# lunarlab-gatech/MorphSym-HGNN

Measured on AMD Instinct MI355X. Metric: graph-windows/sec fwd+bwd, A1-C2 GRF regression, higher is better.
Workload: dtype bf16; 1 GPU; A1-C2 GRF regression (3-D), h=128, L=3, T=150, 8192 windows/GPU, fwd+MSE+bwd, all parameter gradients; global_batch=8192, parallelism=dp1, rccl_ranks=0

## Files before the change

morphsym_hgnn_amd/csrc/mshgnn.hip:

```cpp
#include "mshgnn_slab.hpp"
extern "C" const char* mshgnn_last_error(void) { return g_err.c_str(); }
extern "C" const char* mshgnn_version(void) { return "mshgnn 0.5 (gfx950)"; }
extern "C" int mshgnn_abi_version(void) { return MSHGNN_ABI_VERSION; }
extern "C" size_t mshgnn_struct_size(int which) {
    switch (which) {
        case 0: return sizeof(mshgnn_desc);
        case 1: return sizeof(mshgnn_info);
        case 2: return sizeof(mshgnn_ws_layout);
        case 3: return sizeof(mshgnn_window_desc);
        case 4: return sizeof(mshgnn_kernel_stat);
        default: return 0;
    }
}


template <typename T> __device__ __forceinline__ void prep_one(const PrepArgs& a, int idx, bool with_bias) {
    constexpr int EPC = Prec<T>::EPC, NBV = Prec<T>::NBV;
    const int vec_per_pack = H * H / EPC;
    const int npk = a.pack_n < 0 ? a.n_packs : a.pack_n;
    const int total = npk * vec_per_pack;
    if (idx < total) {
        const int pack = a.pack0 + idx / vec_per_pack, r = idx % vec_per_pack;
        const int gid = pack * vec_per_pack + r;
        const int lane = r % 64, v = (r / 64) % NBV, wv = r / (64 * NBV);
// ... 14 lines not shown
                    else g[i][x] = a.params[pd.src[i] + (int64_t)k * pd.ld + col];
                }
            }
#pragma unroll
        for (int x = 0; x < EPC; ++x) {
            float sum = 0.f;
#pragma unroll
            for (int i = 0; i < 8; ++i) sum += g[i][x];
            out[x] = from_f32<T>(sum);
        }
        T* dst = reinterpret_cast<T*>(a.wpack) + (size_t)gid * EPC;
#pragma unroll
        for (int x = 0; x < EPC; ++x) dst[x] = out[x];
    } else if (with_bias) {
        const int b = idx - total;
        if (b < a.n_biases * H) {
            const BiasDesc bd = a.biases[b / H];
            float s = 0.f;
            for (int i = 0; i < bd.n_src; ++i) s += a.params[bd.src[i] + (b % H)];
            a.bias[b] = s;
        }
    }
}
template <typename T> __global__ void k_prep(PrepArgs a) { prep_one<T>(a, blockIdx.x * blockDim.x + threadIdx.x, true); }


__device__ __forceinline__ u32x4 splice8(u32x4 A, u32x4 B, int n0) {
    const unsigned __int128 a = ((unsigned __int128)(((unsigned long long)A[3] << 32) | A[2]) << 64) | (((unsigned long long)A[1] << 32) | A[0]);
    const unsigned __int128 b = ((unsigned __int128)(((unsigned long long)B[3] << 32) | B[2]) << 64) | (((unsigned long long)B[1] << 32) | B[0]);
    const int sh = 16 * n0;
    const unsigned __int128 r = (a & ((((unsigned __int128)1) << sh) - 1)) | (b << sh);
    return u32x4{(unsigned)r, (unsigned)(r >> 32), (unsigned)(r >> 64), (unsigned)(r >> 96)};
}
template <typename T, bool ALIGNED, bool SERIES = false, int SRC = 0, bool NORM = false> __global__ __launch_bounds__(256) void k_enc_fwd(EncArgs a, SeriesSrc ser, WideSrc wsrc) {
    using P = Prec<T>;
    static_assert(!NORM || SERIES, "standardisation is part of the series gather");
    static_assert(!SERIES || (sizeof(T) == 2 && ALIGNED), "the series gather is a bf16 path");
    static_assert(SRC == 0 || (sizeof(T) == 2 && ALIGNED && !SERIES), "wide source rows: bf16 plan, aligned destination rows");
    constexpr int MB = P::ENC_MB;
    constexpr int VPB = P::ROWS * P::CPR, NIT = VPB / 256 > 0 ? VPB / 256 : 1, BPP = 256 / VPB > 0 ? 256 / VPB : 1;
    extern __shared__ __attribute__((aligned(16))) char smem[];
    const int tid = threadIdx.x, lane = tid & 63, wv = __builtin_amdgcn_readfirstlane(tid >> 6);
    const int lab_blocks = SERIES ? (int)((ser.lab.B + 255) / 256) : 0;
    if constexpr (SERIES) {
        if ((int)blockIdx.x < lab_blocks) {
            const int64_t b = (int64_t)blockIdx.x * 256 + tid;
            if (b < ser.lab.B) window_labels_one(ser.lab, b);
            return;
        }
    }
    const int bid = (int)blockIdx.x - lab_blocks;
    if (bid >= a.wg_prefix[a.n_types]) {
        if constexpr (sizeof(T) == 2 && ALIGNED && !SERIES) prep_one<T>(a.prep, (bid - a.wg_prefix[a.n_types]) * 256 + tid, false);
        return;
    }
    int t = 0;
    while (t + 1 < a.n_types && bid >= a.wg_prefix[t + 1]) ++t;
    const int local = bid - a.wg_prefix[t];
    const int node = a.node_list[a.node_off[t] + (ENC_ORDER ? local % a.nodes[t] : local / a.tiles)], tile = ENC_ORDER ? local / a.nodes[t] : local % a.tiles;
    const bool skip = SERIES && ((a.skip_mask >> (a.tbase[t] + node)) & 1ull) != 0;
    const int w0 = tile * MB * P::ROWS;
    const T* x = reinterpret_cast<const T*>(a.x[t]);
    const int64_t pitch = a.pitch[t];
    const int F = a.width[t], nt = a.tbase[t + 1] - a.tbase[t], nkc = a.nkc[t], vb = a.vb[t];
    const uint8_t* sg = a.signs + a.sign_off[t] + (size_t)node * nkc * H;
    const T* wpack = reinterpret_cast<const T*>(a.wpack);
    const float* bias = a.bias + (size_t)max(a.bias_idx[t], 0) * H;

    typename P::Acc acc[MB];
#pragma unroll
    for (int m = 0; m < MB; ++m) acc_init_bias<T>(acc[m], bias, wv, lane);
    const int c = tid % P::CPR, r0 = (tid % VPB) / P::CPR, sub = tid / VPB;
    typename P::BFrag bf;
    typename P::AFrag af;
    const AOff<T> ao(lane);
    u32x4 v[MB / BPP][NIT];
    u32x4 rawv[(SERIES || SRC) ? MB / BPP : 1][NIT];
    u32x2 wv8[SRC ? MB / BPP : 1][SRC ? SRC : 1];
    const bool unit_ok = SRC == 8 || (F & 1) == 0;
    const int64_t spitch = SRC ? wsrc.pitch[t] : 0;
    int srow[SERIES ? MB / BPP : 1];
    u32x4 vn[NORM ? MB / BPP : 1][2];
    RunStats rsa[NORM ? MB / BPP : 1], rsb[NORM ? MB / BPP : 1];
    int n_n0 = 8; bool n_has_a = false, n_has_b = false;
    __shared__ unsigned long long rp_s[SERIES ? 16 : 1];
    int rfirst = 0, rend = 0;
    if constexpr (SERIES) {
#pragma unroll
        for (int mi = 0; mi < MB / BPP; ++mi) srow[mi] = (int)ser.starts[min(w0 + (mi * BPP + sub) * P::ROWS + r0, a.B - 1)];
        rfirst = ser.rows[2 * (ser.row0[t] + node)]; rend = ser.rows[2 * (ser.row0[t] + node) + 1];
        if (tid < 16) rp_s[tid] = rfirst + tid < rend ? ser.run_ptr[rfirst + tid] : 0ull;
        __syncthreads();
    }
    auto fetch = [&](int kc) {
        const int k0 = kc * H + c * P::EPC;
        const int nvalid = min(P::EPC, F - k0);
        if constexpr (SERIES) {
            const int j = k0 / ser.T, off = k0 - j * ser.T, n0 = min(P::EPC, ser.T - off);
            const bool second = nvalid > n0;
            auto run_ptr_of = [&](int jj) -> unsigned long long { return jj < 16 ? rp_s[jj] : (rfirst + jj < rend ? ser.run_ptr[rfirst + jj] : 0ull); };
            const unsigned long long pa = nvalid > 0 ? run_ptr_of(j) : 0ull, pb = second ? run_ptr_of(j + 1) : 0ull;
            if constexpr (NORM) {
                n_n0 = n0; n_has_a = pa != 0ull; n_has_b = pb != 0ull;
                const u32x4 ones32 = u32x4{0x3f800000u, 0x3f800000u, 0x3f800000u, 0x3f800000u};
#pragma unroll
                for (int mi = 0; mi < MB / BPP; ++mi) {
                    u32x4 a0 = nvalid > 0 ? ones32 : u32x4{0, 0, 0, 0}, a1 = a0;
                    const double* sp2 = ser.stats + ((size_t)min(w0 + (mi * BPP + sub) * P::ROWS + r0, a.B - 1) * ser.n_runs + rfirst + j) * 2;
                    rsa[mi] = RunStats{0.0, 1.0}; rsb[mi] = RunStats{0.0, 1.0};
                    if (pa) {
                        const float* sp = reinterpret_cast<const float*>(pa) + srow[mi] + off;
                        a0 = *reinterpret_cast<const u32x4*>(sp); a1 = *reinterpret_cast<const u32x4*>(sp + 4);
                        const f64x2 sv = *reinterpret_cast<const f64x2*>(sp2);
                        rsa[mi] = RunStats{sv[0], sv[1]};
                    }
                    if (second) {
                        u32x4 b0 = ones32, b1 = ones32;
                        if (pb) {
                            const float* sp = reinterpret_cast<const float*>(pb) + srow[mi];
                            b0 = *reinterpret_cast<const u32x4*>(sp); b1 = *reinterpret_cast<const u32x4*>(sp + 4);
                            const f64x2 sv = *reinterpret_cast<const f64x2*>(sp2 + 2);
                            rsb[mi] = RunStats{sv[0], sv[1]};
                        }
                        splice8f(a0, a1, b0, b1, n0);
                    }
                    vn[mi][0] = a0; vn[mi][1] = a1;
                }
                return;
            }
            const u32x4 ones = u32x4{0x3f803f80u, 0x3f803f80u, 0x3f803f80u, 0x3f803f80u};
#pragma unroll
            for (int mi = 0; mi < MB / BPP; ++mi) {
                u32x4 va = nvalid > 0 ? ones : u32x4{0, 0, 0, 0};
                if (pa) va = *reinterpret_cast<const u32x4*>(reinterpret_cast<const T*>(pa) + srow[mi] + off);
                if (second) {
                    u32x4 vb2 = ones;
                    if (pb) vb2 = *reinterpret_cast<const u32x4*>(reinterpret_cast<const T*>(pb) + srow[mi]);
                    va = splice8(va, vb2, n0);
                }
                v[mi][0] = va;
            }
            return;
        }
        if constexpr (SRC > 0) {
#pragma unroll
            for (int mi = 0; mi < MB / BPP; ++mi) {
                const int w = w0 + (mi * BPP + sub) * P::ROWS + r0;
                const char* row = reinterpret_cast<const char*>(wsrc.p[t]) + ((size_t)min(w, a.B - 1) * nt + node) * spitch * SRC;
                wide_fetch<SRC>(wv8[mi], row, k0, F, unit_ok, w < a.B);
            }
            return;
        }
#pragma unroll
        for (int mi = 0; mi < MB / BPP; ++mi)
#pragma unroll
            for (int it = 0; it < NIT; ++it) {
                const int m = mi * BPP + sub, row = r0 + it * (256 / P::CPR), w = w0 + m * P::ROWS + row;
                if constexpr (ALIGNED) {
                    const T* src = x + ((size_t)min(w, a.B - 1) * nt + node) * pitch + (nvalid > 0 ? k0 : kc * H);
                    v[mi][it] = ld16<ENC_NT>(src);
                } else {
                    v[mi][it] = u32x4{0, 0, 0, 0};
                    if (w < a.B) v[mi][it] = load_chunk<T>(x + ((size_t)w * nt + node) * pitch + k0, nvalid, vb);
                }
            }
    };
    fetch(0);
    for (int kc = 0; kc < nkc; ++kc) {
        const u32x4 sx = sign_xor<T>(sg + kc * H + c * P::EPC);
        const int nv = F - (kc * H + c * P::EPC);
        __syncthreads();
#pragma unroll
        for (int mi = 0; mi < MB / BPP; ++mi)
#pragma unroll
            for (int it = 0; it < NIT; ++it) {
                u32x4 raw;
                if constexpr (SRC > 0) {
                    f32x4 lo4, hi4;
                    wide_to_f32<SRC>(wv8[mi], nv, lo4, hi4);
                    raw = pack_oct(lo4, hi4);
                } else if constexpr (NORM) {
                    u32x4 a0 = vn[mi][0], a1 = vn[mi][1];
                    standardise_oct(a0, a1, n_n0, n_has_a, n_has_b, rsa[mi], rsb[mi]);
                    raw = pack_oct(__builtin_bit_cast(f32x4, a0), __builtin_bit_cast(f32x4, a1));
                    if (kc + 1 == nkc) raw = chunk_keep_first<T>(raw, nv);
                } else
                raw = kc + 1 == nkc ? chunk_keep_first<T>(v[mi][it], nv) : v[mi][it];
                *reinterpret_cast<u32x4*>(smem + lds_chunk<T>(mi * BPP + sub, r0 + it * (256 / P::CPR), c)) = raw ^ sx;
                if constexpr (SERIES || SRC > 0) rawv[mi][it] = raw;
            }
        __syncthreads();
        if (!skip) load_bfrag<T>(bf, wpack, a.pack0[t] + kc, wv, lane);
        if (kc + 1 < nkc) fetch(kc + 1);
        if constexpr (SERIES || SRC > 0) {
#pragma unroll
            for (int mi = 0; mi < MB / BPP; ++mi)
#pragma unroll
                for (int it = 0; it < NIT; ++it) {
                    const int w = w0 + (mi * BPP + sub) * P::ROWS + r0 + it * (256 / P::CPR), k0 = kc * H + c * P::EPC;
                    if (x != nullptr && w < a.B && k0 < (int)pitch) *reinterpret_cast<u32x4*>(const_cast<T*>(x) + ((size_t)w * nt + node) * pitch + k0) = rawv[mi][it];
                }
        }
        if (!skip) {
#pragma unroll
            for (int m = 0; m < MB; ++m) {
                if (w0 + m * P::ROWS < a.B) {
                    load_afrag<T>(af, smem, m, ao);
                    mac(acc[m], af, bf);
                }
            }
        }
    }
    if (skip) return;
    T* x0 = reinterpret_cast<T*>(a.x0);
    const int gnode = a.tbase[t] + node;
#pragma unroll
    for (int m = 0; m < MB; ++m) {
        const int w = w0 + m * P::ROWS + c_win(lane);
        if (w0 + m * P::ROWS < a.B) {
            const unsigned bits = relu_with_bits<T>(acc[m]);
            if (a.mask0) a.mask0[relu_tile_base(gnode, a.B, (w0 + m * P::ROWS) >> 4, wv) + lane] = (uint8_t)bits;
        }
        if (w < a.B) store_oct(x0 + act_idx(w, gnode, a.B) + wv * 32 + c_oct(lane), acc[m].c[0], acc[m].c[1]);
    }
}

struct LayerArgs {
    const void* x_in;
    void* x_out;
    unsigned* maskbits;
    void* hb; void* t1;
    void* dh; void* du;
    const void* x_act;
    const void* wpack; const float* bias; const int* prog;
    int B, NN, n_mlp;
    int dbg;
};

template <typename T>
__device__ __forceinline__ void store_relu_bits(const typename Prec<T>::Acc& acc, unsigned* maskbits, int NN, int n, int w0, int B, int wn, int lane) {
    unsigned bits = 0;
#pragma unroll
    for (int fb = 0; fb < 2; ++fb)
// ... 1404 lines not shown
            p->hp.d = *desc;
        }
        *out = p;
        return MSHGNN_OK;
    }
    int ndev = 0;
    if (hipGetDeviceCount(&ndev) != hipSuccess || ndev == 0) {
        delete p; return set_err(MSHGNN_EHIP, "no HIP device: the MS-HGNN engine has no CPU fallback");
    }
#ifdef MSHGNN_ABLATE
    { const char* e = getenv("MSHGNN_DBG"); p->dbg = e ? atoi(e) : 0; e = getenv("MSHGNN_DBG_GW"); p->dbg_gw = e ? atoi(e) : 0; }
#endif
    HostPlan& hp = p->hp;
    auto up = [&](void** dptr, const void* src, size_t bytes) -> int {
        HIPCHK(hipMalloc(dptr, std::max<size_t>(bytes, 16)));
        if (bytes) HIPCHK(hipMemcpy(*dptr, src, bytes, hipMemcpyHostToDevice));
        return MSHGNN_OK;
    };
    int rc;
    if ((rc = up((void**)&p->d_tables, hp.tables.data(), hp.tables.size() * 4)) != 0 ||
        (rc = up((void**)&p->d_signs, hp.signs.data(), hp.signs.size())) != 0 ||
        (rc = up((void**)&p->d_out_mask, hp.out_mask_f.data(), hp.out_mask_f.size() * 4)) != 0 ||
        (rc = up((void**)&p->d_packs, hp.packs.data(), hp.packs.size() * sizeof(PackDesc))) != 0 ||
        (rc = up((void**)&p->d_biases, hp.biases.data(), hp.biases.size() * sizeof(BiasDesc))) != 0) {
        mshgnn_plan_destroy(p); return rc;
    }
    const int lds = hp.n_blk * hp.blk_bytes;
    if (hp.d.dtype == MSHGNN_BF16X3) {
        p->use_fused = true;
        { const char* et = getenv("MSHGNN_STEP_KERNEL"); p->use_step = !(et && atoi(et) == 0); }
        if ((rc = x3_set_attrs(p))) { mshgnn_plan_destroy(p); return rc; }
    } else if (hp.d.dtype == MSHGNN_F32) {
        if ((rc = set_lds_attr(k_layer_fwd<float>, lds)) || (rc = set_lds_attr(k_layer_bwd<float>, lds)) ||
            (rc = set_lds_attr(k_enc_fwd<float, true>, Prec<float>::ENC_MB * Prec<float>::BLK)) || (rc = set_lds_attr(k_enc_fwd<float, false>, Prec<float>::ENC_MB * Prec<float>::BLK))) { mshgnn_plan_destroy(p); return rc; }
    } else {
        if ((rc = set_lds_attr(k_layer_fwd<__bf16>, lds)) || (rc = set_lds_attr(k_layer_bwd<__bf16>, lds)) ||
            (rc = set_lds_attr(k_enc_fwd<__bf16, true>, Prec<__bf16>::ENC_MB * Prec<__bf16>::BLK)) || (rc = set_lds_attr(k_enc_fwd<__bf16, true, true>, Prec<__bf16>::ENC_MB * Prec<__bf16>::BLK)) || (rc = set_lds_attr(k_enc_fwd<__bf16, true, false, 8>, Prec<__bf16>::ENC_MB * Prec<__bf16>::BLK)) || (rc = set_lds_attr(k_enc_fwd<__bf16, true, false, 4>, Prec<__bf16>::ENC_MB * Prec<__bf16>::BLK)) || (rc = set_lds_attr(k_enc_fwd<__bf16, false>, Prec<__bf16>::ENC_MB * Prec<__bf16>::BLK))) { mshgnn_plan_destroy(p); return rc; }
        const char* e = getenv("MSHGNN_FUSED");
        p->use_fused = hp.fused && !(e && atoi(e) == 0);
        if (p->use_fused) {
            const int flds = (hp.fs_blk + FS_EXTRA_BLK) * Prec<__bf16>::BLK;
            if ((rc = set_lds_attr(k_stack_fwd<__bf16>, flds)) || (rc = set_lds_attr(k_stack_bwd<__bf16>, flds)) || (rc = set_lds_attr(k_stack_step<__bf16>, flds))) { mshgnn_plan_destroy(p); return rc; }
            const char* es = getenv("MSHGNN_SLAB");
            p->use_slab = hp.slab && !(es && atoi(es) == 0);
            p->slab_force = es && atoi(es) == 2;
            { int dev = 0, cus = 256; if (hipGetDevice(&dev) == hipSuccess) (void)hipDeviceGetAttribute(&cus, hipDeviceAttributeMultiprocessorCount, dev); p->n_cu = cus > 0 ? cus : 256; }
            if (p->use_slab && ((rc = set_lds_attr(slab_fwd_kernel(hp), flds)) || (rc = set_lds_attr(slab_bwd_kernel(hp), flds)) ||
                                (rc = set_lds_attr(slab_step_kernel(hp), flds)))) { mshgnn_plan_destroy(p); return rc; }
            { const char* esp = getenv("MSHGNN_SPEC"); p->use_spec = p->use_slab && !(esp && atoi(esp) == 0); }
            if (p->use_spec && (rc = set_spec_attrs(p, flds))) { mshgnn_plan_destroy(p); return rc; }
            { const char* et = getenv("MSHGNN_STEP_KERNEL"); p->use_step = !(et && atoi(et) == 0); }

            { const char* eg = TUNE_ENV("MSHGNN_STAGGER"); p->stagger = eg ? atoi(eg) : 0; }
        }
    }
    *out = p;
    return MSHGNN_OK;
}

extern "C" void mshgnn_plan_destroy(mshgnn_plan* p) {
    if (!p) return;
    gen_destroy(p);
    if (p->d_tables) (void)hipFree(p->d_tables);
    if (p->d_signs) (void)hipFree(p->d_signs);
    if (p->d_out_mask) (void)hipFree(p->d_out_mask);
    if (p->d_packs) (void)hipFree(p->d_packs);
    if (p->d_biases) (void)hipFree(p->d_biases);
    if (p->d_ig_nodes) (void)hipFree(p->d_ig_nodes);
    for (ProfRec& r : p->recs) { (void)hipEventDestroy(r.a); (void)hipEventDestroy(r.b); }
    for (hipEvent_t e : p->free_events) (void)hipEventDestroy(e);
// ... 115 lines not shown
            if (a.pitch[t] < d.type_width[t]) return set_err(MSHGNN_EINVAL, "x_pitch smaller than the feature width");
            a.vb[t] = vec_bytes(a.x[t], a.pitch[t], (int)sizeof(T));
            if (t == 0) a.aligned = 1;
            if (a.vb[t] != 16 || a.pitch[t] % Prec<T>::EPC) a.aligned = 0;
            a.width[t] = d.type_width[t]; a.tbase[t] = hp.type_base[t]; a.nkc[t] = hp.enc_nkc[t];
            a.pack0[t] = hp.pack_enc_base[t]; a.bias_idx[t] = hp.bias_enc[t]; a.sign_off[t] = hp.sign_off[t];
            a.node_off[t] = t == 0 ? 0 : a.node_off[t - 1] + a.nodes[t - 1];
            a.nodes[t] = 0;
            const bool all_rows = series != nullptr && x != nullptr;
            for (int i = 0; i < d.type_nodes[t]; ++i) {
                const bool need = hp.need_n[0][hp.type_base[t] + i];
                if (need || all_rows) a.node_list[a.node_off[t] + a.nodes[t]++] = (unsigned char)i;
                if (!need) a.skip_mask |= 1ull << (hp.type_base[t] + i);
            }
            a.wg_prefix[t + 1] = a.wg_prefix[t] + a.nodes[t] * a.tiles;
        }
        a.tbase[hp.NT] = hp.NN;
        a.wpack = ws + lay.wpack; a.bias = reinterpret_cast<const float*>(ws + lay.bias); a.signs = p->d_signs; a.x0 = ws + lay.x[0];
        a.mask0 = (training && lay.dd[0]) ? reinterpret_cast<uint8_t*>(ws + lay.dd[0]) : nullptr;
        unsigned enc_grid = (unsigned)a.wg_prefix[hp.NT];
        if (embed) {
            PrepArgs lp = pa; lp.pack0 = 0; lp.pack_n = enc_pack0;
            if (a.aligned) { a.prep = lp; a.prep_vecs = enc_pack0 * (H * H / Prec<T>::EPC); enc_grid += (unsigned)((a.prep_vecs + 255) / 256); }
            else {
                ProfScope ps(p, hp.ks_prep, st);
                hipLaunchKernelGGL(k_prep<T>, dim3((unsigned)(((int64_t)enc_pack0 * (H * H / Prec<T>::EPC) + 255) / 256)), dim3(256), 0, st, lp);
            }
        }
        ProfScope ps(p, hp.ks_enc, st);
        if constexpr (sizeof(T) == 2) {
            if (series) {
                if (x && !a.aligned) return set_err(MSHGNN_EINVAL, "the fused window assembly needs 16-byte aligned window rows (pitch a multiple of 8)");
                enc_grid += (unsigned)((series->lab.B + 255) / 256);
                if (series->stats) hipLaunchKernelGGL((k_enc_fwd<T, true, true, 0, true>), dim3(enc_grid), dim3(256), Prec<T>::ENC_MB * Prec<T>::BLK, st, a, *series, WideSrc{});
                else hipLaunchKernelGGL((k_enc_fwd<T, true, true>), dim3(enc_grid), dim3(256), Prec<T>::ENC_MB * Prec<T>::BLK, st, a, *series, WideSrc{});
            } else if (wide) {
                if (x && !a.aligned) return set_err(MSHGNN_EINVAL, "wide source rows: the plan-dtype rows need 16-byte alignment and a pitch that is a multiple of 8");
                if (wide->bytes == 8) hipLaunchKernelGGL((k_enc_fwd<T, true, false, 8>), dim3(enc_grid), dim3(256), Prec<T>::ENC_MB * Prec<T>::BLK, st, a, SeriesSrc{}, *wide);
                else hipLaunchKernelGGL((k_enc_fwd<T, true, false, 4>), dim3(enc_grid), dim3(256), Prec<T>::ENC_MB * Prec<T>::BLK, st, a, SeriesSrc{}, *wide);
            } else if (a.aligned) hipLaunchKernelGGL((k_enc_fwd<T, true>), dim3(enc_grid), dim3(256), Prec<T>::ENC_MB * Prec<T>::BLK, st, a, SeriesSrc{}, WideSrc{});
            else hipLaunchKernelGGL((k_enc_fwd<T, false>), dim3(enc_grid), dim3(256), Prec<T>::ENC_MB * Prec<T>::BLK, st, a, SeriesSrc{}, WideSrc{});
        } else {
            if (wide) return set_err(MSHGNN_EUNSUPPORTED, "wide source rows: not on the fp32 plan (cast the inputs)");
            if (a.aligned) hipLaunchKernelGGL((k_enc_fwd<T, true>), dim3(enc_grid), dim3(256), Prec<T>::ENC_MB * Prec<T>::BLK, st, a, SeriesSrc{}, WideSrc{});
            else hipLaunchKernelGGL((k_enc_fwd<T, false>), dim3(enc_grid), dim3(256), Prec<T>::ENC_MB * Prec<T>::BLK, st, a, SeriesSrc{}, WideSrc{});
        }
    }
    const int tiles = (B + Prec<T>::ROWS - 1) / Prec<T>::ROWS;
    if constexpr (sizeof(T) == 2) {
        if (p->use_fused) {
            StackArgs a{};
            a.tile_in = ws + lay.x[0]; a.ws = ws;
            for (int l = 0; l <= hp.L; ++l) a.x_off[l] = lay.x[l];
            for (int l = 0; l < hp.L; ++l) { a.mask_off[l] = lay.mask[l]; a.hb_off[l] = lay.hb[l]; a.t1_off[l] = lay.t1[l]; a.prog_off[l] = hp.fs_fwd_off[l]; }
            a.wpack = ws + lay.wpack; a.bias = reinterpret_cast<const float*>(ws + lay.bias); a.tables = p->d_tables;
            a.B = B; a.NN = hp.NN; a.L = hp.L; a.training = training;
            a.dbg = p->dbg;
            a.params = params; a.out_mask = p->d_out_mask; a.out = c.out; a.off_dec_w = d.off_dec_w; a.off_dec_b = d.off_dec_b;
            a.node0 = hp.type_base[d.out_type]; a.n_out = d.type_nodes[d.out_type]; a.dout = d.out_channels;
            if (y_fused) {
                a.y = y_fused; a.dec_slabs = reinterpret_cast<float*>(ws + lay.dec_slabs); a.dx_off[hp.L] = lay.dx[hp.L];
                a.inv_n = 1.0f / (float)(c.total_windows() * a.n_out * a.dout);
            } else if (labels_fused) {
                a.labels = labels_fused; a.dec_slabs = reinterpret_cast<float*>(ws + lay.dec_slabs); a.dx_off[hp.L] = lay.dx[hp.L];
                a.inv_n = 1.0f / (float)(c.total_windows() * a.n_out);
            }
            c.dec_done = y_fused || labels_fused;
            a.stamps = stamp_ptr("MSHGNN_STAMPS");
            a.stagger = p->slab_for(tiles) && tiles > p->n_cu ? p->stagger : 0;
            a.stash_nt = training ? stash_nt_for(p->stash_nt_force, B, stash_rows_of(hp), H * (int)sizeof(T)) : 0;
            const bool want_step = p->use_step && c.dec_done;
            bool step_slab = p->slab_for(tiles);
            const bool spec_small = !step_slab && want_step && p->use_slab && p->use_spec && slab_step_spec_kernel(hp, a.stash_nt, nullptr, whole_tiles(B)) != nullptr;
            bool red_front_ok = false, red_back_ok = false; size_t red_back = 0;
            auto red_fits = [&](bool slab) {
                const size_t red_need = (size_t)((slab ? SL_THREADS : LAYER_THREADS) / 64) * DEC_SLAB_FLOATS * sizeof(float);
                const size_t lds_launch = (size_t)((slab ? hp.sl_blk : hp.fs_blk) + FS_EXTRA_BLK) * Prec<T>::BLK;
                red_back = (size_t)(a.node0 + a.n_out) * Prec<T>::BLK;
// ... 556 lines not shown
```

morphsym_hgnn_amd/csrc/mshgnn_device.hpp:

```cpp
#pragma once
#include <type_traits>
#include <hip/hip_runtime.h>

#include <cmath>
#include <cstdio>
#include <cstdlib>
#include <cstring>
#include <string>
#include <vector>

#include "mshgnn_plan.hpp"

using namespace mshgnn;

typedef float f32x4 __attribute__((ext_vector_type(4)));
typedef float f32x2 __attribute__((ext_vector_type(2)));
typedef float f32x16 __attribute__((ext_vector_type(16)));
typedef __bf16 bf16x8 __attribute__((ext_vector_type(8)));
typedef unsigned int u32x4 __attribute__((ext_vector_type(4)));
typedef double f64x2 __attribute__((ext_vector_type(2)));
typedef unsigned int u32x2 __attribute__((ext_vector_type(2)));

#ifndef ENC_NT
#define ENC_NT 0
#endif
#ifndef GW_NT
#define GW_NT 0
#endif
#ifndef ENC_ORDER
#define ENC_ORDER 0
#endif
template <int NT> __device__ __forceinline__ u32x4 ld16(const void* p) {
    if constexpr (NT != 0) return __builtin_nontemporal_load(reinterpret_cast<const u32x4*>(p));
    else return *reinterpret_cast<const u32x4*>(p);
}

inline thread_local std::string g_err;
inline int set_err(int code, const std::string& m) { g_err = m; return code; }
#define HIPCHK(expr)                                                                              \
    do {                                                                                          \
        hipError_t e_ = (expr);                                                                   \
        if (e_ != hipSuccess)                                                                     \
            return set_err(MSHGNN_EHIP, std::string(#expr) + ": " + hipGetErrorString(e_));       \
    } while (0)



#if defined(MSHGNN_GW_STAMPS) && MSHGNN_GW_STAMPS
#define MSHGNN_GW_STAMPS_BUILD 1
#else
#define MSHGNN_GW_STAMPS_BUILD 0
#endif
#ifdef MSHGNN_ABLATE
#define ABL(x) ((x) != 0)
#else
#define ABL(x) (false)
#endif
template <typename T> struct Prec;
template <> struct Prec<float> {
    static constexpr int ROWS = 16, EPC = 4, CPR = 32, RB = 512, NREG = 8, NBV = 16, NAV = 8, HS = 6, BLK = 8192, ENC_MB = 4, WPS = 2;
    using Vec = f32x4;
    struct Acc { f32x4 c[2]; };
    struct AFrag { f32x4 v[8]; };
// ... 439 lines not shown
}

template <typename T> __device__ __forceinline__ u32x4 load_chunk(const T* p, int nvalid, int vb) {
    constexpr int EPC = Prec<T>::EPC;
    u32x4 r = u32x4{0, 0, 0, 0};
    if (nvalid <= 0) return r;
    if (nvalid >= EPC && vb >= 16) return *reinterpret_cast<const u32x4*>(p);
    if (nvalid >= EPC && vb == 8) {
        const u32x2 a = reinterpret_cast<const u32x2*>(p)[0], b = reinterpret_cast<const u32x2*>(p)[1];
        return u32x4{a[0], a[1], b[0], b[1]};
    }
    if (nvalid >= EPC && vb == 4) {
        const unsigned* q = reinterpret_cast<const unsigned*>(p);
        return u32x4{q[0], q[1], q[2], q[3]};
    }
    union { T e[EPC]; u32x4 v; } tmp;
#pragma unroll
    for (int e = 0; e < EPC; ++e) tmp.e[e] = e < nvalid ? p[e] : from_f32<T>(0.f);
    return tmp.v;
}
template <typename T> __device__ __forceinline__ u32x4 chunk_keep_first(u32x4 v, int nv) {
    if constexpr (sizeof(T) == 4) {
#pragma unroll
        for (int e = 0; e < 4; ++e) if (e >= nv) v[e] = 0u;
    } else {
#pragma unroll
        for (int e = 0; e < 4; ++e) {
            const unsigned m = (2 * e < nv ? 0x0000ffffu : 0u) | (2 * e + 1 < nv ? 0xffff0000u : 0u);
            v[e] &= m;
        }
    }
    return v;
}
template <typename T> __device__ __forceinline__ u32x4 sign_xor(const uint8_t* s) {
    if constexpr (sizeof(T) == 4) {
        const unsigned w = *reinterpret_cast<const unsigned*>(s);
        return u32x4{(w & 1u) << 31, ((w >> 8) & 1u) << 31, ((w >> 16) & 1u) << 31, ((w >> 24) & 1u) << 31};
    } else {
        const unsigned w0 = reinterpret_cast<const unsigned*>(s)[0], w1 = reinterpret_cast<const unsigned*>(s)[1];
        return u32x4{((w0 & 1u) << 15) | (((w0 >> 8) & 1u) << 31), (((w0 >> 16) & 1u) << 15) | (((w0 >> 24) & 1u) << 31),
                     ((w1 & 1u) << 15) | (((w1 >> 8) & 1u) << 31), (((w1 >> 16) & 1u) << 15) | (((w1 >> 24) & 1u) << 31)};
    }
}

template <typename T> __device__ __forceinline__ u32x4 chunk_add(u32x4 a, u32x4 b) {
    union U { u32x4 v; T e[Prec<T>::EPC]; } x, y, r;
    x.v = a; y.v = b;
#pragma unroll
    for (int e = 0; e < Prec<T>::EPC; ++e) r.e[e] = from_f32<T>(to_f32(x.e[e]) + to_f32(y.e[e]));
    return r.v;
}
template <typename T> __device__ __forceinline__ u32x4 chunk_mask_pos(u32x4 v, u32x4 act) {
    union U { u32x4 v; T e[Prec<T>::EPC]; } x, y;
    x.v = v; y.v = act;
#pragma unroll
    for (int e = 0; e < Prec<T>::EPC; ++e) if (!(to_f32(y.e[e]) > 0.f)) x.e[e] = from_f32<T>(0.f);
    return x.v;
}
template <typename T> __device__ __forceinline__ u32x4 chunk_mask_bits(u32x4 v, unsigned bits) {
    if constexpr (sizeof(T) == 4) {
#pragma unroll
        for (int e = 0; e < 4; ++e) if (!((bits >> e) & 1u)) v[e] = 0u;
    } else {
#pragma unroll
        for (int e = 0; e < 4; ++e) {
            const int lo = __builtin_amdgcn_sbfe((int)bits, 2 * e, 1), hi = __builtin_amdgcn_sbfe((int)bits, 2 * e + 1, 1);
            v[e] &= (unsigned)((lo & 0xffff) | (hi & (int)0xffff0000));
        }
    }
    return v;
}


template <typename T> __device__ __forceinline__ void load8(const T* p, float (&v)[8]) {
    if constexpr (sizeof(T) == 4) {
// ... 734 lines not shown
```

morphsym_hgnn_amd/csrc/mshgnn_x3.hip:

```cpp
#include "mshgnn_x3_stack.hpp"

__device__ __forceinline__ void prep_one_x3(const PrepArgs& a, int idx, bool with_bias) {
    constexpr int EPC = 8, NBV = 8;
    const int vec_per_pack = H * H / EPC;
    const int npk = a.pack_n < 0 ? a.n_packs : a.pack_n;
    const int total = npk * vec_per_pack;
    if (idx < total) {
        const int pack = a.pack0 + idx / vec_per_pack, r = idx % vec_per_pack;
        const int gid = pack * vec_per_pack + r;
        const int lane = r % 64, v = (r / 64) % NBV, wv = r / (64 * NBV);
        const PackDesc pd = a.packs[pack];
        float g[8][EPC];
#pragma unroll
        for (int i = 0; i < 8; ++i)
#pragma unroll
            for (int x = 0; x < EPC; ++x) {
                const int i16 = lane & 15;
                const int k = 32 * (lane >> 4) + 8 * (v & 3) + x, col = wv * 32 + 8 * (i16 >> 2) + 4 * (v >> 2) + (i16 & 3);
                g[i][x] = 0.f;
                if (i < pd.n_src) {
                    if (pd.orient == 0) { if (k < pd.ncols) g[i][x] = a.params[pd.src[i] + (int64_t)col * pd.ld + pd.col0 + k]; }
                    else g[i][x] = a.params[pd.src[i] + (int64_t)k * pd.ld + col];
                }
            }
// ... 44 lines not shown
    }
    int t = 0;
    while (t + 1 < a.n_types && bid >= a.wg_prefix[t + 1]) ++t;
    const int local = bid - a.wg_prefix[t];
    const int node = a.node_list[a.node_off[t] + (ENC_ORDER ? local % a.nodes[t] : local / a.tiles)], tile = ENC_ORDER ? local / a.nodes[t] : local % a.tiles;
    const bool skip = SERIES && ((a.skip_mask >> (a.tbase[t] + node)) & 1ull) != 0;
    const int w0 = tile * MB * P::ROWS;
    const float* x = reinterpret_cast<const float*>(a.x[t]);
    const int64_t pitch = a.pitch[t];
    const int F = a.width[t], nt = a.tbase[t + 1] - a.tbase[t], nkc = a.nkc[t], vb = a.vb[t];
    const uint8_t* sg = a.signs + a.sign_off[t] + (size_t)node * nkc * H;
    const T16* wpack = reinterpret_cast<const T16*>(a.wpack);
    const float* bias = a.bias + (size_t)max(a.bias_idx[t], 0) * H;

    P::Acc acc[MB];
#pragma unroll
    for (int m = 0; m < MB; ++m) acc_init_bias<T16>(acc[m], bias, wv, lane);
    const int c = tid & 15, r0 = tid >> 4;
    P::BFrag bfh, bfl;
    P::AFrag af;
    const AOff<T16> ao(lane);
    u32x4 v[MB][2];
    u32x2 wv8[SRC ? MB : 1][SRC ? SRC : 1];
    const bool unit_ok = SRC == 8 || (F & 1) == 0;
    const int64_t spitch = SRC ? wsrc.pitch[t] : 0;
    int srow[SERIES ? MB : 1]; int rfirst = 0;
    RunStats rsa[NORM ? MB : 1], rsb[NORM ? MB : 1];
    int n_n0 = 8; bool n_has_a = false, n_has_b = false;
    if constexpr (SERIES) {
#pragma unroll
        for (int m = 0; m < MB; ++m) srow[m] = (int)ser.starts[min(w0 + m * P::ROWS + r0, a.B - 1)];
        rfirst = ser.rows[2 * (ser.row0[t] + node)];
    }
    auto fetch = [&](int kc) {
        const int k0 = kc * H + c * 8;
        const int nv = F - k0;
        if constexpr (SERIES) {
            const int j = k0 / ser.T, off = k0 - j * ser.T, n0 = min(8, ser.T - off);
            const bool second = min(nv, 8) > n0;
            const unsigned long long pa = nv > 0 ? ser.run_ptr[rfirst + j] : 0ull, pb = second ? ser.run_ptr[rfirst + j + 1] : 0ull;
            const u32x4 ones = u32x4{0x3f800000u, 0x3f800000u, 0x3f800000u, 0x3f800000u};
            if constexpr (NORM) { n_n0 = n0; n_has_a = pa != 0ull; n_has_b = pb != 0ull; }
#pragma unroll
            for (int m = 0; m < MB; ++m) {
                u32x4 a0 = nv > 0 ? ones : u32x4{0, 0, 0, 0}, a1 = a0;
                if constexpr (NORM) {
                    const double* sp2 = ser.stats + ((size_t)min(w0 + m * P::ROWS + r0, a.B - 1) * ser.n_runs + rfirst + j) * 2;
                    rsa[m] = RunStats{0.0, 1.0}; rsb[m] = RunStats{0.0, 1.0};
                    if (pa) { const f64x2 sv = *reinterpret_cast<const f64x2*>(sp2); rsa[m] = RunStats{sv[0], sv[1]}; }
                    if (pb) { const f64x2 sv = *reinterpret_cast<const f64x2*>(sp2 + 2); rsb[m] = RunStats{sv[0], sv[1]}; }
                }
                if (pa) {
                    const float* sp = reinterpret_cast<const float*>(pa) + srow[m] + off;
                    a0 = *reinterpret_cast<const u32x4*>(sp); a1 = *reinterpret_cast<const u32x4*>(sp + 4);
                }
                if (second) {
                    u32x4 b0 = ones, b1 = ones;
                    if (pb) {
                        const float* sp = reinterpret_cast<const float*>(pb) + srow[m];
                        b0 = *reinterpret_cast<const u32x4*>(sp); b1 = *reinterpret_cast<const u32x4*>(sp + 4);
                    }
                    splice8f(a0, a1, b0, b1, n0);
                }
                v[m][0] = a0; v[m][1] = a1;
            }
            return;
        }
        if constexpr (SRC > 0) {
#pragma unroll
            for (int m = 0; m < MB; ++m) {
                const int w = w0 + m * P::ROWS + r0;
                const char* row = reinterpret_cast<const char*>(wsrc.p[t]) + ((size_t)min(w, a.B - 1) * nt + node) * spitch * SRC;
                wide_fetch<SRC>(wv8[m], row, k0, F, unit_ok, w < a.B);
            }
            return;
        }
#pragma unroll
        for (int m = 0; m < MB; ++m) {
            const int w = w0 + m * P::ROWS + r0;
            if constexpr (ALIGNED) {
                const float* src = x + ((size_t)min(w, a.B - 1) * nt + node) * pitch;
                v[m][0] = ld16<ENC_NT>(src + (nv > 0 ? k0 : kc * H));
                v[m][1] = ld16<ENC_NT>(src + (nv > 4 ? k0 + 4 : kc * H));
            } else {
                v[m][0] = u32x4{0, 0, 0, 0}; v[m][1] = u32x4{0, 0, 0, 0};
                if (w < a.B) {
                    const float* src = x + ((size_t)w * nt + node) * pitch + k0;
                    v[m][0] = load_chunk<float>(src, nv, vb);
                    v[m][1] = load_chunk<float>(src + 4, nv - 4, vb);
                }
            }
        }
    };
    fetch(0);
    for (int kc = 0; kc < nkc; ++kc) {
        const u32x4 sxa = sign_xor<float>(sg + kc * H + c * 8), sxb = sign_xor<float>(sg + kc * H + c * 8 + 4);
        const int nv = F - (kc * H + c * 8);
        __syncthreads();
#pragma unroll
        for (int m = 0; m < MB; ++m) {
            u32x4 fa = v[m][0], fb = v[m][1];
            if constexpr (SRC > 0) {
                f32x4 lo4, hi4;
                wide_to_f32<SRC>(wv8[m], nv, lo4, hi4);
                fa = __builtin_bit_cast(u32x4, lo4); fb = __builtin_bit_cast(u32x4, hi4);
            } else
            {
                if constexpr (NORM) standardise_oct(fa, fb, n_n0, n_has_a, n_has_b, rsa[m], rsb[m]);
                if (kc + 1 == nkc) { fa = chunk_keep_first<float>(fa, nv); fb = chunk_keep_first<float>(fb, nv - 4); }
            }
            if constexpr (SERIES || SRC > 0) {
                const int w = w0 + m * P::ROWS + r0, k0 = kc * H + c * 8;
                if (x != nullptr && w < a.B) {
                    float* dst = const_cast<float*>(x) + ((size_t)w * nt + node) * pitch + k0;
                    if (k0 < (int)pitch) *reinterpret_cast<u32x4*>(dst) = fa;
                    if (k0 + 4 < (int)pitch) *reinterpret_cast<u32x4*>(dst + 4) = fb;
                }
            }
            fa ^= sxa; fb ^= sxb;
            u32x4 hi, lo;
            split_oct(__builtin_bit_cast(f32x4, fa), __builtin_bit_cast(f32x4, fb), hi, lo);
            *reinterpret_cast<u32x4*>(smem + lds_chunk<T16>(m, r0, c)) = hi;
            *reinterpret_cast<u32x4*>(smem + lds_chunk<T16>(MB + m, r0, c)) = lo;
        }
        __syncthreads();
        if (!skip) {
            load_bfrag<T16>(bfh, wpack, a.pack0[t] + kc, wv, lane);
            load_bfrag<T16>(bfl, wpack, n_img + a.pack0[t] + kc, wv, lane);
        }
        if (kc + 1 < nkc) fetch(kc + 1);
        if (!skip) {
#pragma unroll
            for (int m = 0; m < MB; ++m) {
                if (w0 + m * P::ROWS < a.B) {
                    load_afrag<T16>(af, smem, m, ao);
                    mac(acc[m], af, bfh);
                    mac(acc[m], af, bfl);
                    load_afrag<T16>(af, smem, MB + m, ao);
                    mac(acc[m], af, bfh);
                }
            }
        }
    }
    if (skip) return;
    T16* x0 = reinterpret_cast<T16*>(a.x0);
    const int gnode = a.tbase[t] + node;
#pragma unroll
    for (int m = 0; m < MB; ++m) {
        const int w = w0 + m * P::ROWS + c_win(lane);
        if (w0 + m * P::ROWS < a.B) {
            const unsigned bits = relu_with_bits<T16>(acc[m]);
            if (a.mask0) a.mask0[relu_tile_base(gnode, a.B, (w0 + m * P::ROWS) >> 4, wv) + lane] = (uint8_t)bits;
        }
        if (w < a.B) {
            u32x4 hi, lo;
            split_oct(acc[m].c[0], acc[m].c[1], hi, lo);
            T16* q = x0 + x3_idx(w, gnode, a.B) + wv * 32 + c_oct(lane);
            *reinterpret_cast<u32x4*>(q) = hi;
            *reinterpret_cast<u32x4*>(q + H) = lo;
        }
    }
}

template <bool ALIAS> __global__ __launch_bounds__(LAYER_THREADS, 2) void k_stack_fwd_x3(StackArgs a) {
    extern __shared__ __attribute__((aligned(16))) char smem[];
    stack_fwd_x3_body<ALIAS, false>(a, smem);
}

__global__ __launch_bounds__(LAYER_THREADS, 2) void k_stack_bwd_x3(StackArgs a) {
    extern __shared__ __attribute__((aligned(16))) char smem[];
    stack_bwd_x3_body<false>(a, smem);
}

using SpecSelectorX3 = StackKernelX3 (*)(const HostPlan& hp, int kind, const char** name);
// ... 690 lines not shown
```

Before: 45.14 million windows/s.

## Double-buffer encoder LDS staging and prefetch weight fragments and sign words

Restructures the bf16 encoder forward loop to double-buffer the LDS A-tile, so staging of chunk kc+1 overlaps the MACs on chunk kc and one barrier per iteration is removed. Sign-flip words are now loaded together with each chunk fetch, and the x3 encoder prefetches B fragments for the next chunk right after the current MACs. It also precomputes per-row byte offsets for the aligned fetch and requests a minimum of four waves per EU for the plain bf16 path. The costs are double the LDS per block, which can lower occupancy, and more register pressure.

```diff
diff --git a/morphsym_hgnn_amd/csrc/mshgnn.hip b/morphsym_hgnn_amd/csrc/mshgnn.hip
--- a/morphsym_hgnn_amd/csrc/mshgnn.hip
+++ b/morphsym_hgnn_amd/csrc/mshgnn.hip
@@ -70,7 +70,10 @@
     const unsigned __int128 r = (a & ((((unsigned __int128)1) << sh) - 1)) | (b << sh);
     return u32x4{(unsigned)r, (unsigned)(r >> 32), (unsigned)(r >> 64), (unsigned)(r >> 96)};
 }
-template <typename T, bool ALIGNED, bool SERIES = false, int SRC = 0, bool NORM = false> __global__ __launch_bounds__(256) void k_enc_fwd(EncArgs a, SeriesSrc ser, WideSrc wsrc) {
+template <typename T, bool NORM> constexpr bool enc_pipe() { return ENC_PIPE != 0 && sizeof(T) == 2 && !NORM; }
+template <typename T, bool NORM = false> constexpr int enc_lds_bytes() { return Prec<T>::ENC_MB * Prec<T>::BLK * (enc_pipe<T, NORM>() ? 2 : 1); }
+template <typename T, bool SERIES, int SRC> constexpr int enc_min_waves() { return sizeof(T) == 2 && !SERIES && SRC == 0 ? 4 : 1; }
+template <typename T, bool ALIGNED, bool SERIES = false, int SRC = 0, bool NORM = false> __global__ __launch_bounds__(256) __attribute__((amdgpu_waves_per_eu(enc_min_waves<T, SERIES, SRC>()))) void k_enc_fwd(EncArgs a, SeriesSrc ser, WideSrc wsrc) {
     using P = Prec<T>;
     static_assert(!NORM || SERIES, "standardisation is part of the series gather");
     static_assert(!SERIES || (sizeof(T) == 2 && ALIGNED), "the series gather is a bf16 path");
@@ -130,9 +133,15 @@
         if (tid < 16) rp_s[tid] = rfirst + tid < rend ? ser.run_ptr[rfirst + tid] : 0ull;
         __syncthreads();
     }
+    const char* xrow0 = reinterpret_cast<const char*>(x + ((size_t)min(w0 + r0, a.B - 1) * nt + node) * pitch);
+    unsigned xoff[MB];
+#pragma unroll
+    for (int m = 0; m < MB; ++m) xoff[m] = (unsigned)(min(w0 + m * P::ROWS + r0, a.B - 1) - min(w0 + r0, a.B - 1)) * (unsigned)(nt * pitch * sizeof(T));
+    unsigned sgw[2] = {0u, 0u};
     auto fetch = [&](int kc) {
         const int k0 = kc * H + c * P::EPC;
         const int nvalid = min(P::EPC, F - k0);
+        if constexpr (enc_pipe<T, NORM>()) { sgw[0] = reinterpret_cast<const unsigned*>(sg + k0)[0]; sgw[1] = reinterpret_cast<const unsigned*>(sg + k0)[1]; }
         if constexpr (SERIES) {
             const int j = k0 / ser.T, off = k0 - j * ser.T, n0 = min(P::EPC, ser.T - off);
             const bool second = nvalid > n0;
@@ -194,7 +203,9 @@
 #pragma unroll
             for (int it = 0; it < NIT; ++it) {
                 const int m = mi * BPP + sub, row = r0 + it * (256 / P::CPR), w = w0 + m * P::ROWS + row;
-                if constexpr (ALIGNED) {
+                if constexpr (ALIGNED && enc_pipe<T, NORM>()) {
+                    v[mi][it] = ld16<ENC_NT>(xrow0 + (size_t)(unsigned)opaque((int)xoff[mi]) + (size_t)(nvalid > 0 ? k0 : kc * H) * sizeof(T));
+                } else if constexpr (ALIGNED) {
                     const T* src = x + ((size_t)min(w, a.B - 1) * nt + node) * pitch + (nvalid > 0 ? k0 : kc * H);
                     v[mi][it] = ld16<ENC_NT>(src);
                 } else {
@@ -203,11 +214,8 @@
                 }
             }
     };
-    fetch(0);
-    for (int kc = 0; kc < nkc; ++kc) {
-        const u32x4 sx = sign_xor<T>(sg + kc * H + c * P::EPC);
+    auto stage = [&](int kc, char* sm, const u32x4 sx) {
         const int nv = F - (kc * H + c * P::EPC);
-        __syncthreads();
 #pragma unroll
         for (int mi = 0; mi < MB / BPP; ++mi)
 #pragma unroll
@@ -224,12 +232,11 @@
                     if (kc + 1 == nkc) raw = chunk_keep_first<T>(raw, nv);
                 } else
                 raw = kc + 1 == nkc ? chunk_keep_first<T>(v[mi][it], nv) : v[mi][it];
-                *reinterpret_cast<u32x4*>(smem + lds_chunk<T>(mi * BPP + sub, r0 + it * (256 / P::CPR), c)) = raw ^ sx;
+                *reinterpret_cast<u32x4*>(sm + lds_chunk<T>(mi * BPP + sub, r0 + it * (256 / P::CPR), c)) = raw ^ sx;
                 if constexpr (SERIES || SRC > 0) rawv[mi][it] = raw;
             }
-        __syncthreads();
-        if (!skip) load_bfrag<T>(bf, wpack, a.pack0[t] + kc, wv, lane);
-        if (kc + 1 < nkc) fetch(kc + 1);
+    };
+    auto put_rows = [&](int kc) {
         if constexpr (SERIES || SRC > 0) {
 #pragma unroll
             for (int mi = 0; mi < MB / BPP; ++mi)
@@ -239,14 +246,54 @@
                     if (x != nullptr && w < a.B && k0 < (int)pitch) *reinterpret_cast<u32x4*>(const_cast<T*>(x) + ((size_t)w * nt + node) * pitch + k0) = rawv[mi][it];
                 }
         }
-        if (!skip) {
-#pragma unroll
-            for (int m = 0; m < MB; ++m) {
-                if (w0 + m * P::ROWS < a.B) {
-                    load_afrag<T>(af, smem, m, ao);
-                    mac(acc[m], af, bf);
-                }
-            }
+    };
+    auto macs = [&](const char* sm) {
+#pragma unroll
+        for (int m = 0; m < MB; ++m) {
+            if (w0 + m * P::ROWS < a.B) {
+                load_afrag<T>(af, sm, m, ao);
+                mac(acc[m], af, bf);
+            }
+        }
+    };
+    if constexpr (enc_pipe<T, NORM>()) {
+        constexpr int STAGE = MB * P::BLK;
+        fetch(0);
+        if (!skip) load_bfrag<T>(bf, wpack, a.pack0[t], wv, lane);
+        if (nkc > 0) stage(0, smem, sign_xor_words<T>(sgw[0], sgw[1]));
+        if (nkc > 1) {
+            fetch(1);
+            put_rows(0);
+            __syncthreads();
+            int kc = 0;
+            for (; kc + 2 < nkc; ++kc) {
+                if (!skip) { macs(smem + (kc & 1) * STAGE); load_bfrag<T>(bf, wpack, a.pack0[t] + kc + 1, wv, lane); }
+                stage(kc + 1, smem + ((kc + 1) & 1) * STAGE, sign_xor_words<T>(sgw[0], sgw[1]));
+                fetch(kc + 2);
+                put_rows(kc + 1);
+                __syncthreads();
+            }
+            if (!skip) { macs(smem + (kc & 1) * STAGE); load_bfrag<T>(bf, wpack, a.pack0[t] + kc + 1, wv, lane); }
+            stage(kc + 1, smem + ((kc + 1) & 1) * STAGE, sign_xor_words<T>(sgw[0], sgw[1]));
+            put_rows(kc + 1);
+            __syncthreads();
+            if (!skip) macs(smem + ((kc + 1) & 1) * STAGE);
+        } else if (nkc > 0) {
+            put_rows(0);
+            __syncthreads();
+            if (!skip) macs(smem);
+        }
+    } else {
+        fetch(0);
+        for (int kc = 0; kc < nkc; ++kc) {
+            const u32x4 sx = sign_xor<T>(sg + kc * H + c * P::EPC);
+            __syncthreads();
+            stage(kc, smem, sx);
+            __syncthreads();
+            if (!skip) load_bfrag<T>(bf, wpack, a.pack0[t] + kc, wv, lane);
+            if (kc + 1 < nkc) fetch(kc + 1);
+            put_rows(kc);
+            if (!skip) macs(smem);
         }
     }
     if (skip) return;
@@ -1717,10 +1764,10 @@
         if ((rc = x3_set_attrs(p))) { mshgnn_plan_destroy(p); return rc; }
     } else if (hp.d.dtype == MSHGNN_F32) {
         if ((rc = set_lds_attr(k_layer_fwd<float>, lds)) || (rc = set_lds_attr(k_layer_bwd<float>, lds)) ||
-            (rc = set_lds_attr(k_enc_fwd<float, true>, Prec<float>::ENC_MB * Prec<float>::BLK)) || (rc = set_lds_attr(k_enc_fwd<float, false>, Prec<float>::ENC_MB * Prec<float>::BLK))) { mshgnn_plan_destroy(p); return rc; }
+            (rc = set_lds_attr(k_enc_fwd<float, true>, enc_lds_bytes<float>())) || (rc = set_lds_attr(k_enc_fwd<float, false>, enc_lds_bytes<float>()))) { mshgnn_plan_destroy(p); return rc; }
     } else {
         if ((rc = set_lds_attr(k_layer_fwd<__bf16>, lds)) || (rc = set_lds_attr(k_layer_bwd<__bf16>, lds)) ||
-            (rc = set_lds_attr(k_enc_fwd<__bf16, true>, Prec<__bf16>::ENC_MB * Prec<__bf16>::BLK)) || (rc = set_lds_attr(k_enc_fwd<__bf16, true, true>, Prec<__bf16>::ENC_MB * Prec<__bf16>::BLK)) || (rc = set_lds_attr(k_enc_fwd<__bf16, true, false, 8>, Prec<__bf16>::ENC_MB * Prec<__bf16>::BLK)) || (rc = set_lds_attr(k_enc_fwd<__bf16, true, false, 4>, Prec<__bf16>::ENC_MB * Prec<__bf16>::BLK)) || (rc = set_lds_attr(k_enc_fwd<__bf16, false>, Prec<__bf16>::ENC_MB * Prec<__bf16>::BLK))) { mshgnn_plan_destroy(p); return rc; }
+            (rc = set_lds_attr(k_enc_fwd<__bf16, true>, enc_lds_bytes<__bf16>())) || (rc = set_lds_attr(k_enc_fwd<__bf16, true, true>, enc_lds_bytes<__bf16>())) || (rc = set_lds_attr(k_enc_fwd<__bf16, true, false, 8>, enc_lds_bytes<__bf16>())) || (rc = set_lds_attr(k_enc_fwd<__bf16, true, false, 4>, enc_lds_bytes<__bf16>())) || (rc = set_lds_attr(k_enc_fwd<__bf16, false>, enc_lds_bytes<__bf16>()))) { mshgnn_plan_destroy(p); return rc; }
         const char* e = getenv("MSHGNN_FUSED");
         p->use_fused = hp.fused && !(e && atoi(e) == 0);
         if (p->use_fused) {
@@ -1902,18 +1949,18 @@
             if (series) {
                 if (x && !a.aligned) return set_err(MSHGNN_EINVAL, "the fused window assembly needs 16-byte aligned window rows (pitch a multiple of 8)");
                 enc_grid += (unsigned)((series->lab.B + 255) / 256);
-                if (series->stats) hipLaunchKernelGGL((k_enc_fwd<T, true, true, 0, true>), dim3(enc_grid), dim3(256), Prec<T>::ENC_MB * Prec<T>::BLK, st, a, *series, WideSrc{});
-                else hipLaunchKernelGGL((k_enc_fwd<T, true, true>), dim3(enc_grid), dim3(256), Prec<T>::ENC_MB * Prec<T>::BLK, st, a, *series, WideSrc{});
+                if (series->stats) hipLaunchKernelGGL((k_enc_fwd<T, true, true, 0, true>), dim3(enc_grid), dim3(256), (enc_lds_bytes<T, true>()), st, a, *series, WideSrc{});
+                else hipLaunchKernelGGL((k_enc_fwd<T, true, true>), dim3(enc_grid), dim3(256), enc_lds_bytes<T>(), st, a, *series, WideSrc{});
             } else if (wide) {
                 if (x && !a.aligned) return set_err(MSHGNN_EINVAL, "wide source rows: the plan-dtype rows need 16-byte alignment and a pitch that is a multiple of 8");
-                if (wide->bytes == 8) hipLaunchKernelGGL((k_enc_fwd<T, true, false, 8>), dim3(enc_grid), dim3(256), Prec<T>::ENC_MB * Prec<T>::BLK, st, a, SeriesSrc{}, *wide);
-                else hipLaunchKernelGGL((k_enc_fwd<T, true, false, 4>), dim3(enc_grid), dim3(256), Prec<T>::ENC_MB * Prec<T>::BLK, st, a, SeriesSrc{}, *wide);
-            } else if (a.aligned) hipLaunchKernelGGL((k_enc_fwd<T, true>), dim3(enc_grid), dim3(256), Prec<T>::ENC_MB * Prec<T>::BLK, st, a, SeriesSrc{}, WideSrc{});
-            else hipLaunchKernelGGL((k_enc_fwd<T, false>), dim3(enc_grid), dim3(256), Prec<T>::ENC_MB * Prec<T>::BLK, st, a, SeriesSrc{}, WideSrc{});
+                if (wide->bytes == 8) hipLaunchKernelGGL((k_enc_fwd<T, true, false, 8>), dim3(enc_grid), dim3(256), enc_lds_bytes<T>(), st, a, SeriesSrc{}, *wide);
+                else hipLaunchKernelGGL((k_enc_fwd<T, true, false, 4>), dim3(enc_grid), dim3(256), enc_lds_bytes<T>(), st, a, SeriesSrc{}, *wide);
+            } else if (a.aligned) hipLaunchKernelGGL((k_enc_fwd<T, true>), dim3(enc_grid), dim3(256), enc_lds_bytes<T>(), st, a, SeriesSrc{}, WideSrc{});
+            else hipLaunchKernelGGL((k_enc_fwd<T, false>), dim3(enc_grid), dim3(256), enc_lds_bytes<T>(), st, a, SeriesSrc{}, WideSrc{});
         } else {
             if (wide) return set_err(MSHGNN_EUNSUPPORTED, "wide source rows: not on the fp32 plan (cast the inputs)");
-            if (a.aligned) hipLaunchKernelGGL((k_enc_fwd<T, true>), dim3(enc_grid), dim3(256), Prec<T>::ENC_MB * Prec<T>::BLK, st, a, SeriesSrc{}, WideSrc{});
-            else hipLaunchKernelGGL((k_enc_fwd<T, false>), dim3(enc_grid), dim3(256), Prec<T>::ENC_MB * Prec<T>::BLK, st, a, SeriesSrc{}, WideSrc{});
+            if (a.aligned) hipLaunchKernelGGL((k_enc_fwd<T, true>), dim3(enc_grid), dim3(256), enc_lds_bytes<T>(), st, a, SeriesSrc{}, WideSrc{});
+            else hipLaunchKernelGGL((k_enc_fwd<T, false>), dim3(enc_grid), dim3(256), enc_lds_bytes<T>(), st, a, SeriesSrc{}, WideSrc{});
         }
     }
     const int tiles = (B + Prec<T>::ROWS - 1) / Prec<T>::ROWS;
diff --git a/morphsym_hgnn_amd/csrc/mshgnn_device.hpp b/morphsym_hgnn_amd/csrc/mshgnn_device.hpp
--- a/morphsym_hgnn_amd/csrc/mshgnn_device.hpp
+++ b/morphsym_hgnn_amd/csrc/mshgnn_device.hpp
@@ -29,6 +29,9 @@
 #endif
 #ifndef ENC_ORDER
 #define ENC_ORDER 0
+#endif
+#ifndef ENC_PIPE
+#define ENC_PIPE 1
 #endif
 template <int NT> __device__ __forceinline__ u32x4 ld16(const void* p) {
     if constexpr (NT != 0) return __builtin_nontemporal_load(reinterpret_cast<const u32x4*>(p));
@@ -534,15 +537,14 @@
     }
     return v;
 }
+template <typename T> __device__ __forceinline__ u32x4 sign_xor_words(unsigned w0, unsigned w1) {
+    if constexpr (sizeof(T) == 4) return u32x4{(w0 & 1u) << 31, ((w0 >> 8) & 1u) << 31, ((w0 >> 16) & 1u) << 31, ((w0 >> 24) & 1u) << 31};
+    else return u32x4{((w0 & 1u) << 15) | (((w0 >> 8) & 1u) << 31), (((w0 >> 16) & 1u) << 15) | (((w0 >> 24) & 1u) << 31),
+                      ((w1 & 1u) << 15) | (((w1 >> 8) & 1u) << 31), (((w1 >> 16) & 1u) << 15) | (((w1 >> 24) & 1u) << 31)};
+}
 template <typename T> __device__ __forceinline__ u32x4 sign_xor(const uint8_t* s) {
-    if constexpr (sizeof(T) == 4) {
-        const unsigned w = *reinterpret_cast<const unsigned*>(s);
-        return u32x4{(w & 1u) << 31, ((w >> 8) & 1u) << 31, ((w >> 16) & 1u) << 31, ((w >> 24) & 1u) << 31};
-    } else {
-        const unsigned w0 = reinterpret_cast<const unsigned*>(s)[0], w1 = reinterpret_cast<const unsigned*>(s)[1];
-        return u32x4{((w0 & 1u) << 15) | (((w0 >> 8) & 1u) << 31), (((w0 >> 16) & 1u) << 15) | (((w0 >> 24) & 1u) << 31),
-                     ((w1 & 1u) << 15) | (((w1 >> 8) & 1u) << 31), (((w1 >> 16) & 1u) << 15) | (((w1 >> 24) & 1u) << 31)};
-    }
+    if constexpr (sizeof(T) == 4) return sign_xor_words<T>(*reinterpret_cast<const unsigned*>(s), 0u);
+    else return sign_xor_words<T>(reinterpret_cast<const unsigned*>(s)[0], reinterpret_cast<const unsigned*>(s)[1]);
 }
 
 template <typename T> __device__ __forceinline__ u32x4 chunk_add(u32x4 a, u32x4 b) {
diff --git a/morphsym_hgnn_amd/csrc/mshgnn_x3.hip b/morphsym_hgnn_amd/csrc/mshgnn_x3.hip
--- a/morphsym_hgnn_amd/csrc/mshgnn_x3.hip
+++ b/morphsym_hgnn_amd/csrc/mshgnn_x3.hip
@@ -100,9 +100,16 @@
         for (int m = 0; m < MB; ++m) srow[m] = (int)ser.starts[min(w0 + m * P::ROWS + r0, a.B - 1)];
         rfirst = ser.rows[2 * (ser.row0[t] + node)];
     }
+    constexpr bool PIPE = ENC_PIPE != 0;
+    unsigned sgw[2] = {0u, 0u};
+    auto frags = [&](int kc) {
+        load_bfrag<T16>(bfh, wpack, a.pack0[t] + kc, wv, lane);
+        load_bfrag<T16>(bfl, wpack, n_img + a.pack0[t] + kc, wv, lane);
+    };
     auto fetch = [&](int kc) {
         const int k0 = kc * H + c * 8;
         const int nv = F - k0;
+        if constexpr (PIPE) { sgw[0] = reinterpret_cast<const unsigned*>(sg + k0)[0]; sgw[1] = reinterpret_cast<const unsigned*>(sg + k0)[1]; }
         if constexpr (SERIES) {
             const int j = k0 / ser.T, off = k0 - j * ser.T, n0 = min(8, ser.T - off);
             const bool second = min(nv, 8) > n0;
@@ -161,8 +168,9 @@
         }
     };
     fetch(0);
+    if (PIPE && !skip) frags(0);
     for (int kc = 0; kc < nkc; ++kc) {
-        const u32x4 sxa = sign_xor<float>(sg + kc * H + c * 8), sxb = sign_xor<float>(sg + kc * H + c * 8 + 4);
+        const u32x4 sxa = PIPE ? sign_xor_words<float>(sgw[0], 0u) : sign_xor<float>(sg + kc * H + c * 8), sxb = PIPE ? sign_xor_words<float>(sgw[1], 0u) : sign_xor<float>(sg + kc * H + c * 8 + 4);
         const int nv = F - (kc * H + c * 8);
         __syncthreads();
 #pragma unroll
@@ -192,10 +200,7 @@
             *reinterpret_cast<u32x4*>(smem + lds_chunk<T16>(MB + m, r0, c)) = lo;
         }
         __syncthreads();
-        if (!skip) {
-            load_bfrag<T16>(bfh, wpack, a.pack0[t] + kc, wv, lane);
-            load_bfrag<T16>(bfl, wpack, n_img + a.pack0[t] + kc, wv, lane);
-        }
+        if (!PIPE && !skip) frags(kc);
         if (kc + 1 < nkc) fetch(kc + 1);
         if (!skip) {
 #pragma unroll
@@ -208,6 +213,7 @@
                     mac(acc[m], af, bfh);
                 }
             }
+            if (PIPE && kc + 1 < nkc) frags(kc + 1);
         }
     }
     if (skip) return;
```

Result: no change. 45.09 million windows/s (-0.1%).
